# lucidrains/ring-attention-pytorch

Hardware: AMD Instinct MI355X
Metric: attn_tflops (higher is better)
Workload: dtype bf16; 1 GPU; model=ring_flash_attn (non-causal, d_head 64), global_batch=1, seq_len=8192, seq_per_gpu=8192, heads=8, kv_heads=8, d_head=64, parallelism=ring1, hipgraph=True

## Files before the change

ring_attention_amd/csrc/attn_bwd.hip:

```cpp

#include <hip/hip_runtime.h>
#include <hip/hip_bf16.h>
#include <cstdint>

#include "attn_common.h"

namespace ring_attn {

template <int D>
struct DqLds {
    static constexpr int KVB = kvblk(D);
    __align__(16) __bf16 k[2][KVB * D];
    __align__(16) __bf16 v[2][KVB * D];
    unsigned char kmask[2][KVB];
};

template <int D, bool SOFTCLAMP, bool PAIRED, bool BIAS = false>
__global__ __launch_bounds__(512, 2)
void attn_bwd_dq_kernel(BwdParams p) {
    constexpr int DBLK = D / 32;
    constexpr int KSTEPS = D / 16;
    constexpr int DQ_KVBLK = kvblk(D);
    constexpr int DQ_NBLK = DQ_KVBLK / 32;

    __shared__ DqLds<D> lds;

    const int tid = threadIdx.x;
    const int lane = tid & 63;
    const int wid = tid >> 6;
    const int l31 = lane & 31;
    const int lhi = lane >> 5;

    const int bh = blockIdx.y;
    const int b = bh / p.h;
    const int h = bh % p.h;
    const int hk = h % p.hk;

    const int n_pit = PAIRED
        ? (p.paired - 1 - (int)blockIdx.x == (int)blockIdx.x ? 1 : 2) : 1;
    for (int pit = 0; pit < n_pit; ++pit) {
    const int qtile = PAIRED
        ? (pit == 0 ? (int)blockIdx.x : p.paired - 1 - (int)blockIdx.x)
        : (p.desc ? p.desc[(long)blockIdx.x * 3] : (int)blockIdx.x);
    if (PAIRED && pit == 1) {
        __syncthreads();
    }

    auto dq_body = [&]() {
    const BwdParams P = p;
    const long i = (long)qtile * ROWS_WG + wid * 32 + l31;
    const bool row_valid = i < P.nq;
    const long ic = row_valid ? i : 0;

    const __bf16* qbase = (const __bf16*)P.q + ((long)b * P.nq + ic) * P.h * D + (long)h * D;
    const __bf16* dobase = (const __bf16*)P.dout + ((long)b * P.nq + ic) * P.h * D + (long)h * D;
    bf16x8 qf[KSTEPS], dof[KSTEPS];
    #pragma unroll
    for (int ks = 0; ks < KSTEPS; ++ks) {
        qf[ks] = *(const bf16x8*)(qbase + ks * 16 + lhi * 8);
        dof[ks] = *(const bf16x8*)(dobase + ks * 16 + lhi * 8);
    }
    const float lse_i = P.lse[((long)b * P.h + h) * P.nq + ic] * LOG2E;
    const float delta_i = P.delta[((long)b * P.h + h) * P.nq + ic];

    f32x16 dq_acc[DBLK];
    #pragma unroll
    for (int db = 0; db < DBLK; ++db) dq_acc[db] = f32x16{};

    const Mask M = mask_of(P);
    const long wg_i_min = (long)qtile * ROWS_WG;
    const long wg_i_max = min((long)(qtile + 1) * ROWS_WG, P.nq) - 1;
    const long wg_q_min = M.qpos(wg_i_min);
    const long wg_q_max = M.qpos(wg_i_max);
    const long qpos_i = M.qpos(i);
    TileRange tr = M.kv_tile_range(wg_i_min, wg_i_max, P.nk, DQ_KVBLK);
    if (P.split > 1) tr = split_share(tr, P.split, (int)blockIdx.z);
    if (!PAIRED && P.desc)
        tr = {P.desc[(long)blockIdx.x * 3 + 1], P.desc[(long)blockIdx.x * 3 + 2]};
    const int t_lo = tr.lo, t_hi = tr.hi;

    constexpr int CH = D * 2 / 16;
    constexpr int KCHUNKS = DQ_KVBLK * CH;
    constexpr int KREGS = (KCHUNKS + 511) / 512;
    const __bf16* kbase = (const __bf16*)P.k + ((long)b * P.nk) * P.hk * D + (long)hk * D;
    const __bf16* vbase = (const __bf16*)P.v + ((long)b * P.nk) * P.hk * D + (long)hk * D;
    const unsigned char* mbase = P.kmask ? (const unsigned char*)P.kmask + (long)b * P.nk : nullptr;

    const long kv_row_stride = (long)P.hk * D;
    const long tile_stride = DQ_KVBLK * kv_row_stride;
    const __bf16* kptr = kbase + (long)t_lo * tile_stride
        + (tid / CH) * kv_row_stride + (tid % CH) * 8;
    const __bf16* vptr = vbase + (long)t_lo * tile_stride
        + (tid / CH) * kv_row_stride + (tid % CH) * 8;
    long j0_next = (long)t_lo * DQ_KVBLK;

    uint4 kst[KREGS], vst[KREGS];
    unsigned char mst = 1;

    auto load_tile = [&]() {
        const long j0 = j0_next;
        const long jmax = min(j0 + DQ_KVBLK, P.nk) - 1;
        const bool full = jmax - j0 == DQ_KVBLK - 1;
        #pragma unroll
        for (int r = 0; r < KREGS; ++r) {
            int c = tid + r * 512;
            if (c < KCHUNKS) {
                long off = (long)(r * (512 / CH)) * kv_row_stride;
                bool okr = full || (j0 + c / CH) <= jmax;
                kst[r] = okr ? *(const uint4*)(kptr + off) : uint4{0, 0, 0, 0};
                vst[r] = okr ? *(const uint4*)(vptr + off) : uint4{0, 0, 0, 0};
            }
        }
        if (mbase && tid < DQ_KVBLK)
            mst = (j0 + tid <= jmax) ? mbase[j0 + tid] : 0;
        kptr += tile_stride; vptr += tile_stride;
        j0_next += DQ_KVBLK;
    };

    auto write_tile = [&](int par) {
        #pragma unroll
        for (int r = 0; r < KREGS; ++r) {
            int c = tid + r * 512;
            if (c < KCHUNKS) {
                int row = c / CH, ch = c % CH;
                *(uint4*)(lds.k[par] + row * D + swz<D / 8>(row, ch) * 8) = kst[r];
                *(uint4*)(lds.v[par] + row * D + swz<D / 8>(row, ch) * 8) = vst[r];
            }
        }
        if (mbase && tid < DQ_KVBLK) lds.kmask[par][tid] = mst;
    };

    const float scale2 = P.scale * LOG2E;
    if (t_lo < t_hi) {
        load_tile();
        write_tile(t_lo & 1);
        if (t_lo + 1 < t_hi) load_tile();
    }

    for (int t = t_lo; t < t_hi; ++t) {
        const int par = t & 1;
        const long j0 = (long)t * DQ_KVBLK;
        const long jmax = min(j0 + DQ_KVBLK, P.nk) - 1;
        const bool full_tile = !BIAS &&
            (jmax - j0 == DQ_KVBLK - 1) &&
            M.uncut(wg_q_min, wg_q_max, j0, jmax) &&
            !P.kmask;

        __syncthreads();

        alignas(16) uint32_t pk[DQ_NBLK * 8];
        __builtin_amdgcn_s_setprio(1);
        #pragma unroll
        for (int kb = 0; kb < DQ_NBLK; ++kb) {
            f32x16 s = f32x16{}, dp = f32x16{};
            int krow = kb * 32 + l31;
            #pragma unroll
            for (int ks = 0; ks < KSTEPS; ++ks) {
                int chunk = ks * 2 + lhi;
                bf16x8 kfr = *(const bf16x8*)(lds.k[par] + krow * D + swz<D / 8>(krow, chunk) * 8);
                bf16x8 vfr = *(const bf16x8*)(lds.v[par] + krow * D + swz<D / 8>(krow, chunk) * 8);
                s = __builtin_amdgcn_mfma_f32_32x32x16_bf16(kfr, qf[ks], s, 0, 0, 0);
                dp = __builtin_amdgcn_mfma_f32_32x32x16_bf16(vfr, dof[ks], dp, 0, 0, 0);
            }
            if (full_tile && row_valid) {
                #pragma unroll
                for (int x2 = 0; x2 < 8; ++x2) {
                    float dse[2];
                    #pragma unroll
                    for (int e = 0; e < 2; ++e) {
                        int r = 2 * x2 + e;
                        float x, dtanh = 1.f;
                        if constexpr (SOFTCLAMP) {
                            float inv_v = __builtin_amdgcn_rcpf(P.softclamp_value);
                            float th = fast_tanhf(s[r] * P.scale * inv_v);
                            x = P.softclamp_value * th * LOG2E;
                            dtanh = 1.f - th * th;
                        } else {
                            x = __builtin_fmaf(s[r], scale2, -lse_i);
                        }
                        float pv = __builtin_amdgcn_exp2f(SOFTCLAMP ? x - lse_i : x);
                        dse[e] = pv * (dp[r] - delta_i);
                        if constexpr (SOFTCLAMP) dse[e] *= dtanh;
                    }
                    pk[kb * 8 + x2] = pack_bf16x2(dse[0], dse[1]);
                }
            } else {
                #pragma unroll
                for (int x2 = 0; x2 < 8; ++x2) {
                    float dse[2];
                    #pragma unroll
                    for (int e = 0; e < 2; ++e) {
                        int r = 2 * x2 + e;
                        long jj = j0 + kb * 32 + (r & 3) + 8 * (r >> 2) + 4 * lhi;
                        float x, dtanh = 1.f;
                        if constexpr (SOFTCLAMP) {
                            float inv_v = __builtin_amdgcn_rcpf(P.softclamp_value);
                            float th = fast_tanhf(s[r] * P.scale * inv_v);
                            x = P.softclamp_value * th * LOG2E;
                            dtanh = 1.f - th * th;
                        } else {
                            x = s[r] * scale2;
                        }
                        bool ok = row_valid && jj <= jmax;
                        if constexpr (BIAS) {
                            if (ok) {
                                const long bi = P.bias_mat
                                    ? (((long)b * P.h + h) * P.nq + ic) * P.nk + jj
                                    : ((long)b * P.h + h) * P.nk + jj;
                                x += P.bias[bi] * LOG2E;
                            }
                        }
                        ok = M.attends(qpos_i, jj, ok);
                        if (P.kmask) ok = ok && lds.kmask[par][jj - j0];
                        float pv = ok ? __builtin_amdgcn_exp2f(
                            SOFTCLAMP ? x - lse_i : x - lse_i) : 0.f;
                        dse[e] = pv * (dp[r] - delta_i);
                        if constexpr (SOFTCLAMP) dse[e] *= dtanh;
                    }
                    pk[kb * 8 + x2] = pack_bf16x2(dse[0], dse[1]);
                }
            }
        }
        __builtin_amdgcn_s_setprio(0);

        if (t + 1 < t_hi) write_tile(par ^ 1);
        if (t + 2 < t_hi) load_tile();

        {
            const int f15 = lane & 15;
            const int g16 = (lane >> 4) & 1;
            const unsigned kb_lds = (unsigned)(uintptr_t)
                (__attribute__((address_space(3))) __bf16*)lds.k[par];
            __builtin_amdgcn_s_setprio(1);
            unsigned long long ktr[DBLK][DQ_NBLK * 2][2];
            #pragma unroll
            for (int db = 0; db < DBLK; ++db) {
                const int dg = db * 32 + g16 * 16 + 4 * (f15 & 3);
                #pragma unroll
                for (int ks = 0; ks < DQ_NBLK * 2; ++ks) {
                    #pragma unroll
                    for (int half = 0; half < 2; ++half) {
                        const int kv = ks * 16 + 4 * lhi + 8 * half + (f15 >> 2);
                        const int c = (dg / 8) ^ (kv & (CH < 8 ? CH - 1 : 7));
                        const unsigned a = kb_lds
                            + (unsigned)(kv * (D * 2) + c * 16 + (dg % 8) * 2);
                        asm volatile("ds_read_b64_tr_b16 %0, %1"
                                     : "=&v"(ktr[db][ks][half]) : "v"(a) : "memory");
                    }
                }
            }
            asm volatile("s_waitcnt lgkmcnt(0)" ::: "memory");
            __builtin_amdgcn_sched_barrier(0);
            #pragma unroll
            for (int db = 0; db < DBLK; ++db)
                #pragma unroll
                for (int ks = 0; ks < DQ_NBLK * 2; ++ks) {
                    bf16x8 ktf;
                    *(unsigned long long*)&ktf = ktr[db][ks][0];
                    *((unsigned long long*)&ktf + 1) = ktr[db][ks][1];
                    dq_acc[db] = __builtin_amdgcn_mfma_f32_32x32x16_bf16(
                        ktf, *(const bf16x8*)(pk + 4 * ks), dq_acc[db], 0, 0, 0);
                }
            __builtin_amdgcn_s_setprio(0);
        }
    }

    if (!row_valid) return;
    #pragma unroll
    for (int db = 0; db < DBLK; ++db) dq_acc[db] *= P.scale;
    if (P.dq_bf) {
        __bf16* dqb = (__bf16*)P.dq_bf + ((long)b * P.nq + i) * P.h * D + (long)h * D;
        #pragma unroll
        for (int db = 0; db < DBLK; ++db)
            #pragma unroll
            for (int g = 0; g < 4; ++g) {
                f32x4 v4 = {dq_acc[db][4 * g], dq_acc[db][4 * g + 1],
                            dq_acc[db][4 * g + 2], dq_acc[db][4 * g + 3]};
                *(bf16x4*)(dqb + db * 32 + 8 * g + 4 * lhi) =
                    __builtin_convertvector(v4, bf16x4);
            }
        return;
    }
    float* dqp = P.dq + ((long)b * P.nq + i) * P.h * D + (long)h * D;
    #pragma unroll
    for (int db = 0; db < DBLK; ++db)
        #pragma unroll
        for (int r = 0; r < 16; ++r) {
            int d = db * 32 + (r & 3) + 8 * (r >> 2) + 4 * lhi;
            if (P.split > 1 || P.desc) atomicAdd(dqp + d, dq_acc[db][r]);
            else if (P.accumulate) dqp[d] += dq_acc[db][r];
            else dqp[d] = dq_acc[db][r];
        }
    };
    dq_body();
    }
}

static constexpr int KVROWS_WAVE = 32;
static_assert(ROWS_WG == 8 * KVROWS_WAVE);

template <int D, int QT>
struct DkvLds {
    __align__(16) __bf16 q[2][QT * D];
    __align__(16) __bf16 qt[2][D * QT];
    __align__(16) __bf16 do_[2][QT * D];
    __align__(16) __bf16 dot[2][D * QT];
    __align__(16) float lse[2][QT];
    __align__(16) float delta[2][QT];
};


template <int D, int QT, bool SOFTCLAMP, bool PAIRED, bool BIAS = false>
__global__ __launch_bounds__(512, 2)
void attn_bwd_dkv_kernel(BwdParams p) {
    static_assert(D % 32 == 0 && QT % 32 == 0);
    constexpr int DBLK = D / 32;
    constexpr int KSTEPS = D / 16;
    constexpr int QBLKS = QT / 32;
    constexpr int TM = (QT / 8 - 1) < 7 ? (QT / 8 - 1) : 7;

    __shared__ DkvLds<D, QT> lds;

    constexpr bool FRAME = (D == 64);
    constexpr bool PREFETCH = (D == 64);

    const int n_pit = PAIRED
        ? (p.paired - 1 - (int)blockIdx.x == (int)blockIdx.x ? 1 : 2) : 1;
    for (int pit = 0; pit < n_pit; ++pit) {
    const int kvtile_wg = PAIRED
        ? (pit == 0 ? (int)blockIdx.x : p.paired - 1 - (int)blockIdx.x)
        : (p.desc ? p.desc[(long)blockIdx.x * 3] : (int)blockIdx.x);
    if (PAIRED && pit == 1) {
        __syncthreads();
    }

    auto dkv_body = [&](int kvtile_arg, unsigned long long kernarg) {
    const BwdParams P = [&] {
        if constexpr (FRAME) {
            BwdParams kp = kernarg_params<BwdParams>(kernarg);
            kp.q = as_global(kp.q);         kp.k = as_global(kp.k);
            kp.v = as_global(kp.v);         kp.dout = as_global(kp.dout);
            kp.kmask = as_global(kp.kmask); kp.lse = as_global(kp.lse);
            kp.delta = as_global(kp.delta); kp.dk = as_global(kp.dk);
            kp.dv = as_global(kp.dv);       kp.dk_bf = as_global(kp.dk_bf);
            kp.dv_bf = as_global(kp.dv_bf); kp.bias = as_global(kp.bias);
            kp.desc = as_global(kp.desc);
            return kp;
        } else {
            return p;
        }
    }();
    const int kvtile = uniform<FRAME>(kvtile_arg);
    const int tid = threadIdx.x;
    const int lane = tid & 63;
    const int wid = uniform<FRAME>(tid >> 6);
    const int l31 = lane & 31;
    const int lhi = lane >> 5;
    const int bhk = blockIdx.y;
    const int b = bhk / P.hk;
    const int hkh = bhk % P.hk;

    const long j0_wg = (long)kvtile * ROWS_WG;
    const long jmax = min(j0_wg + ROWS_WG, P.nk) - 1;
    const long j = j0_wg + wid * KVROWS_WAVE + l31;
    const bool col_valid = j <= jmax;
    const long jc = col_valid ? j : j0_wg;

    const __bf16* kb = (const __bf16*)P.k + ((long)b * P.nk + jc) * P.hk * D + (long)hkh * D;
    const __bf16* vb = (const __bf16*)P.v + ((long)b * P.nk + jc) * P.hk * D + (long)hkh * D;
    bf16x8 kf[KSTEPS], vf[KSTEPS];
    #pragma unroll
    for (int ks = 0; ks < KSTEPS; ++ks) {
        kf[ks] = *(const bf16x8*)(kb + ks * 16 + lhi * 8);
        vf[ks] = *(const bf16x8*)(vb + ks * 16 + lhi * 8);
    }
    unsigned char kmask_own = 1;
    if (P.kmask) kmask_own = col_valid ? ((const unsigned char*)P.kmask)[(long)b * P.nk + j] : 0;

    f32x16 dv_acc[DBLK], dk_acc[DBLK];
    #pragma unroll
    for (int db = 0; db < DBLK; ++db) { dv_acc[db] = f32x16{}; dk_acc[db] = f32x16{}; }
    const float scale2 = P.scale * LOG2E;

    const Mask M = mask_of(P);

    if constexpr (FRAME) __builtin_amdgcn_s_waitcnt(0x0F70);

    for (int g = 0; g < P.group; ++g) {
        if (g > 0) __syncthreads();
        const int h = hkh + g * P.hk;
        const float* lse_row = P.lse + ((long)b * P.h + h) * P.nq;
        const float* delta_row = P.delta + ((long)b * P.h + h) * P.nq;
        const __bf16* qg = (const __bf16*)P.q + ((long)b * P.nq) * P.h * D + (long)h * D;
        const __bf16* dog = (const __bf16*)P.dout + ((long)b * P.nq) * P.h * D + (long)h * D;

        TileRange tr = M.q_tile_range(j0_wg, jmax, P.nq, QT);
        if (P.split > 1) tr = split_share(tr, P.split, (int)blockIdx.z);
        if (!PAIRED && P.desc)
            tr = {uniform<FRAME>(P.desc[(long)blockIdx.x * 3 + 1]),
                  uniform<FRAME>(P.desc[(long)blockIdx.x * 3 + 2])};
        const int t0 = tr.lo, t1 = tr.hi;

        constexpr int CH = D * 2 / 16;
        constexpr int QCHUNKS = QT * CH;
        constexpr int QREGS = (QCHUNKS + 511) / 512;
        constexpr int TPAIRS = (QT / 2) * (D / 8);
        constexpr int TREGS = (TPAIRS + 511) / 512;
        uint4 qst[QREGS], dost[QREGS];
        bf16x8 qtv_a[TREGS], qtv_b[TREGS], dov_a[TREGS], dov_b[TREGS];
        float lse_st = 0.f, delta_st = 0.f;
        long t_next = t0;

        const unsigned qrow_bytes = (unsigned)(P.h * D) * 2u;
        auto ld16 = [](const __bf16* base, unsigned boff) {
            return *(const uint4*)((const char*)base + boff);
        };
        auto ld8h = [](const __bf16* base, unsigned boff) {
            return *(const bf16x8*)((const char*)base + boff);
        };
        auto tile_rows = [&](long tile) {
            return (int)(min((tile + 1) * QT, P.nq) - tile * QT);
        };
        auto load_qtile = [&](int tid) {
            const long i0 = t_next * QT;
            const int last = tile_rows(t_next) - 1;
            const __bf16* qtile = qg + i0 * P.h * D;
            const __bf16* dotile = dog + i0 * P.h * D;
            #pragma unroll
            for (int r = 0; r < QREGS; ++r) {
                int c = tid + r * 512;
                if (c < QCHUNKS) {
                    int lr = min(c / CH, last);
                    int ch = c % CH;
                    unsigned off = (unsigned)lr * qrow_bytes + ch * 16;
                    qst[r] = ld16(qtile, off);
                    dost[r] = ld16(dotile, off);
                }
            }
            #pragma unroll
            for (int r = 0; r < TREGS; ++r) {
                int c = tid + r * 512;
                if (c < TPAIRS) {
                    int jp = c % (QT / 2);
                    int d0 = (c / (QT / 2)) * 8;
                    unsigned offa = (unsigned)min(jp * 2, last) * qrow_bytes + d0 * 2;
                    unsigned offb = (unsigned)min(jp * 2 + 1, last) * qrow_bytes + d0 * 2;
                    qtv_a[r] = ld8h(qtile, offa);
                    qtv_b[r] = ld8h(qtile, offb);
                    dov_a[r] = ld8h(dotile, offa);
                    dov_b[r] = ld8h(dotile, offb);
                }
            }
            if (tid < QT) {
                long gi = i0 + min(tid, last);
                lse_st = lse_row[gi];
                delta_st = delta_row[gi];
            }
            ++t_next;
        };

        auto write_qtile = [&](int par, int tid, long tile) {
            const int rows = tile_rows(tile);
            if (rows < QT) {
                #pragma unroll
                for (int r = 0; r < QREGS; ++r)
                    if ((tid + r * 512) / CH >= rows) {
                        qst[r] = uint4{0, 0, 0, 0};
                        dost[r] = uint4{0, 0, 0, 0};
                    }
                #pragma unroll
                for (int r = 0; r < TREGS; ++r) {
                    int la = ((tid + r * 512) % (QT / 2)) * 2;
                    if (la >= rows) { qtv_a[r] = bf16x8{}; dov_a[r] = bf16x8{}; }
                    if (la + 1 >= rows) { qtv_b[r] = bf16x8{}; dov_b[r] = bf16x8{}; }
                }
            }
            #pragma unroll
            for (int r = 0; r < QREGS; ++r) {
                int c = tid + r * 512;
                if (c < QCHUNKS) {
                    int row = c / CH, ch = c % CH;
                    *(uint4*)(lds.q[par] + row * D + swz<D / 8>(row, ch) * 8) = qst[r];
                    *(uint4*)(lds.do_[par] + row * D + swz<D / 8>(row, ch) * 8) = dost[r];
                }
            }
            #pragma unroll
            for (int r = 0; r < TREGS; ++r) {
                int c = tid + r * 512;
                if (c < TPAIRS) {
                    int jp = kperm_pair(c % (QT / 2));
                    int d0 = (c / (QT / 2)) * 8;
                    static_assert((TM << 4) < QT * 2 && (D * QT * 2) % (QT * 2) == 0);
                    const unsigned base = par * (D * QT * 2) + d0 * QT * 2 + jp * 4;
                    #pragma unroll
                    for (int e = 0; e < 8; ++e) {
                        unsigned byte_off = (base ^ ((e & TM) << 4)) + e * QT * 2;
                        __bf16 pq[2] = {qtv_a[r][e], qtv_b[r][e]};
                        __bf16 pd[2] = {dov_a[r][e], dov_b[r][e]};
                        *(uint32_t*)((char*)lds.qt[0] + byte_off) = *(uint32_t*)pq;
                        *(uint32_t*)((char*)lds.dot[0] + byte_off) = *(uint32_t*)pd;
                    }
                }
            }
            if (tid < QT) {
                const bool okl = tid < rows;
                lds.lse[par][tid] = okl ? lse_st * LOG2E : 0.f;
                lds.delta[par][tid] = okl ? delta_st : 0.f;
            }
        };

        if (t0 < t1) {
            load_qtile(tid);
            write_qtile(t0 & 1, tid, t0);
            if (t0 + 1 < t1) load_qtile(tid);
        }

        for (int t = t0; t < t1; ++t) {
            const int par = t & 1;
            const long i0 = (long)t * QT;
            const long imax = min(i0 + QT, P.nq) - 1;
            const bool full_tile = !BIAS &&
                (imax - i0 == QT - 1) &&
                M.uncut(M.qpos(i0), M.qpos(imax), j0_wg, jmax) &&
                !P.kmask;

            bf16x8 qa[KSTEPS], da[KSTEPS], doa[2 * DBLK], qta[2 * DBLK];
            auto read_sdp = [&](int qb) {
                #pragma unroll
                for (int ks = 0; ks < KSTEPS; ++ks) {
                    int qrow = qb * 32 + l31;
                    int chunk = ks * 2 + lhi;
                    qa[ks] = *(const bf16x8*)(lds.q[par] + qrow * D + swz<D / 8>(qrow, chunk) * 8);
                    da[ks] = *(const bf16x8*)(lds.do_[par] + qrow * D + swz<D / 8>(qrow, chunk) * 8);
                }
            };
            auto read_dvdk = [&](int qb) {
                #pragma unroll
                for (int db = 0; db < DBLK; ++db)
                    #pragma unroll
                    for (int half = 0; half < 2; ++half) {
                        int qk = qb * 2 + half;
                        int drow = db * 32 + l31;
                        int ch = qk * 2 + lhi;
                        doa[db * 2 + half] = *(const bf16x8*)(lds.dot[par] + drow * QT +
                                                              ((ch ^ (drow & TM))) * 8);
                        qta[db * 2 + half] = *(const bf16x8*)(lds.qt[par] + drow * QT +
                                                              ((ch ^ (drow & TM))) * 8);
                    }
            };

            const int rows_m1 = (int)(imax - i0);
            int lhi4 = 4 * lhi;
            asm volatile("" : "+v"(lhi4));
            long qp_lane = M.qpos(i0 + lhi4);
            asm volatile("" : "+v"(qp_lane));

            __syncthreads();

            if constexpr (PREFETCH) {
                read_sdp(0);
                __builtin_amdgcn_sched_barrier(0);
            }

            int tid_l = tid;
            if constexpr (FRAME) asm volatile("" : "+v"(tid_l));
            if (t + 1 < t1) write_qtile(par ^ 1, tid_l, t + 1);
            if (t + 2 < t1) load_qtile(tid_l);

            #pragma unroll
            for (int qb = 0; qb < QBLKS; ++qb) {
                f32x16 s2 = f32x16{}, dp = f32x16{};
                if constexpr (!PREFETCH) read_sdp(qb);
                #pragma unroll
                for (int ks = 0; ks < KSTEPS; ++ks) {
                    s2 = __builtin_amdgcn_mfma_f32_32x32x16_bf16(qa[ks], kf[ks], s2, 0, 0, 0);
                    dp = __builtin_amdgcn_mfma_f32_32x32x16_bf16(da[ks], vf[ks], dp, 0, 0, 0);
                }
                f32x4 lse_g0 = f32x4{}, delta_g0 = f32x4{};
                if constexpr (PREFETCH) {
                    lse_g0 = *(const f32x4*)(lds.lse[par] + qb * 32 + 4 * lhi);
                    delta_g0 = *(const f32x4*)(lds.delta[par] + qb * 32 + 4 * lhi);
                    read_dvdk(qb);
                    __builtin_amdgcn_sched_barrier(0);
                }

                alignas(16) uint32_t p_pk[8], ds_pk[8];
                if (full_tile && col_valid) {
                    #pragma unroll
                    for (int x2 = 0; x2 < 8; ++x2) {
                        float pe[2], dse[2];
                        f32x4 lse4, delta4;
                        if (PREFETCH && (x2 >> 1) == 0) {
                            lse4 = lse_g0;
                            delta4 = delta_g0;
                        } else {
                            int base = qb * 32 + 8 * (x2 >> 1) + 4 * lhi;
                            lse4 = *(const f32x4*)(lds.lse[par] + base);
                            delta4 = *(const f32x4*)(lds.delta[par] + base);
                        }
                        #pragma unroll
                        for (int e = 0; e < 2; ++e) {
                            int r = 2 * x2 + e;
                            float x, dtanh = 1.f;
                            if constexpr (SOFTCLAMP) {
                                float inv_v = __builtin_amdgcn_rcpf(P.softclamp_value);
                                float th = fast_tanhf(s2[r] * P.scale * inv_v);
                                x = P.softclamp_value * th * LOG2E;
                                dtanh = 1.f - th * th;
                            } else {
                                x = __builtin_fmaf(s2[r], scale2, -lse4[r & 3]);
                            }
                            float pv = __builtin_amdgcn_exp2f(SOFTCLAMP ? x - lse4[r & 3] : x);
                            pe[e] = pv;
                            dse[e] = pv * (dp[r] - delta4[r & 3]);
                            if constexpr (SOFTCLAMP) dse[e] *= dtanh;
                        }
                        p_pk[x2] = pack_bf16x2(pe[0], pe[1]);
                        ds_pk[x2] = pack_bf16x2(dse[0], dse[1]);
                    }
                } else {
                    #pragma unroll
                    for (int x2 = 0; x2 < 8; ++x2) {
                        float pe[2], dse[2];
                        f32x4 lse4, delta4;
                        if (PREFETCH && (x2 >> 1) == 0) {
                            lse4 = lse_g0;
                            delta4 = delta_g0;
                        } else {
                            int base = qb * 32 + 8 * (x2 >> 1) + 4 * lhi;
                            lse4 = *(const f32x4*)(lds.lse[par] + base);
                            delta4 = *(const f32x4*)(lds.delta[par] + base);
                        }
                        #pragma unroll
                        for (int e = 0; e < 2; ++e) {
                            int r = 2 * x2 + e;
                            const int cr = qb * 32 + (r & 3) + 8 * (r >> 2);
                            const int qloc = cr + lhi4;
                            float x, dtanh = 1.f;
                            if constexpr (SOFTCLAMP) {
                                float inv_v = __builtin_amdgcn_rcpf(P.softclamp_value);
                                float th = fast_tanhf(s2[r] * P.scale * inv_v);
                                x = P.softclamp_value * th * LOG2E;
                                dtanh = 1.f - th * th;
                            } else {
                                x = s2[r] * scale2;
                            }
                            bool ok = col_valid && qloc <= rows_m1;
                            if constexpr (BIAS) {
                                if (ok) {
                                    const long i = i0 + qloc;
                                    const long bi = P.bias_mat
                                        ? (((long)b * P.h + h) * P.nq + i) * P.nk + j
                                        : ((long)b * P.h + h) * P.nk + j;
                                    x += P.bias[bi] * LOG2E;
                                }
                            }
                            ok = M.attends(qp_lane + (long)cr * M.q_stride, j, ok);
                            if (P.kmask) ok = ok && kmask_own;
                            float pv = ok ? __builtin_amdgcn_exp2f(x - lse4[r & 3]) : 0.f;
                            pe[e] = pv;
                            dse[e] = pv * (dp[r] - delta4[r & 3]);
                            if constexpr (SOFTCLAMP) dse[e] *= dtanh;
                        }
                        p_pk[x2] = pack_bf16x2(pe[0], pe[1]);
                        ds_pk[x2] = pack_bf16x2(dse[0], dse[1]);
                    }
                }

                if constexpr (PREFETCH) {
                    if (qb + 1 < QBLKS) {
                        read_sdp(qb + 1);
                        __builtin_amdgcn_sched_barrier(0);
                    }
                } else {
                    read_dvdk(qb);
                }
                #pragma unroll
                for (int db = 0; db < DBLK; ++db)
                    #pragma unroll
                    for (int half = 0; half < 2; ++half) {
                        dv_acc[db] = __builtin_amdgcn_mfma_f32_32x32x16_bf16(
                            doa[db * 2 + half], *(const bf16x8*)(p_pk + 4 * half), dv_acc[db], 0, 0, 0);
                        dk_acc[db] = __builtin_amdgcn_mfma_f32_32x32x16_bf16(
                            *(const bf16x8*)(ds_pk + 4 * half), qta[db * 2 + half], dk_acc[db], 0, 0, 0);
                    }
            }
        }
    }

    #pragma unroll
    for (int db = 0; db < DBLK; ++db) dk_acc[db] *= P.scale;

    if (P.dk_bf) {
        constexpr int ECH = D / 8;
        __bf16* stg_dk = (__bf16*)&lds;
        __bf16* stg_dv = stg_dk + ROWS_WG * D;
        static_assert(sizeof(DkvLds<D, QT>) >= 2 * ROWS_WG * D * sizeof(__bf16));
        const int wrow0 = wid * KVROWS_WAVE;
        const long orow_stride = (long)P.hk * D;
        __bf16* dkb = (__bf16*)P.dk_bf + ((long)b * P.nk) * orow_stride + (long)hkh * D;
        __bf16* dvb = (__bf16*)P.dv_bf + ((long)b * P.nk) * orow_stride + (long)hkh * D;
        __syncthreads();
        #pragma unroll
        for (int db = 0; db < DBLK; ++db)
            #pragma unroll
            for (int r = 0; r < 16; ++r) {
                int row = wrow0 + (r & 3) + 8 * (r >> 2) + 4 * lhi;
                int d = db * 32 + l31;
                stg_dk[row * D + swz<ECH>(row, d / 8) * 8 + (d & 7)] = (__bf16)dk_acc[db][r];
            }
        {
            const int row = wrow0 + l31;
            #pragma unroll
            for (int db = 0; db < DBLK; ++db)
                #pragma unroll
                for (int g = 0; g < 4; ++g) {
                    f32x4 v4 = {dv_acc[db][4 * g], dv_acc[db][4 * g + 1],
                                dv_acc[db][4 * g + 2], dv_acc[db][4 * g + 3]};
                    *(bf16x4*)(stg_dv + row * D + swz<ECH>(row, db * 4 + g) * 8 + 4 * lhi) =
                        __builtin_convertvector(v4, bf16x4);
                }
        }
        __syncthreads();
        #pragma unroll
        for (int c = lane; c < KVROWS_WAVE * ECH; c += 64) {
            int row = wrow0 + c / ECH, ch = c % ECH;
            long kvrow = j0_wg + row;
            if (kvrow <= jmax) {
                int so = row * D + swz<ECH>(row, ch) * 8;
                *(uint4*)(dkb + kvrow * orow_stride + ch * 8) = *(const uint4*)(stg_dk + so);
                *(uint4*)(dvb + kvrow * orow_stride + ch * 8) = *(const uint4*)(stg_dv + so);
            }
        }
    } else {
        float* dkb = P.dk + (((long)b * P.hk + hkh) * P.nk) * D;
        #pragma unroll
        for (int db = 0; db < DBLK; ++db)
            #pragma unroll
            for (int r = 0; r < 16; ++r) {
                long kvrow = j0_wg + wid * KVROWS_WAVE + (r & 3) + 8 * (r >> 2) + 4 * lhi;
                int d = db * 32 + l31;
                if (kvrow <= jmax) {
                    float* dst = dkb + kvrow * D + d;
                    if (P.split > 1 || P.desc) atomicAdd(dst, dk_acc[db][r]);
                    else if (P.accumulate) *dst += dk_acc[db][r];
                    else *dst = dk_acc[db][r];
                }
            }
        float* dvb = P.dv + (((long)b * P.hk + hkh) * D) * P.nk;
        if (col_valid)
        #pragma unroll
        for (int db = 0; db < DBLK; ++db)
            #pragma unroll
            for (int r = 0; r < 16; ++r) {
                int d = db * 32 + (r & 3) + 8 * (r >> 2) + 4 * lhi;
                float* dst = dvb + (long)d * P.nk + j;
                if (P.split > 1 || P.desc) atomicAdd(dst, dv_acc[db][r]);
                else if (P.accumulate) *dst += dv_acc[db][r];
                else *dst = dv_acc[db][r];
            }
    }
    };
    if constexpr (FRAME) noinline_call(dkv_body, kvtile_wg, kernarg_address());
    else dkv_body(kvtile_wg, 0ull);
    }
}

void launch_attn_bwd_dq(const BwdParams& p, int head_dim, hipStream_t stream) {
    dim3 block(512);
    int z = p.split > 1 ? p.split : 1;
    long qt_ = ceil_div(p.nq, ROWS_WG);
    if (p.desc) qt_ = p.n_units;
    else if (p.paired) qt_ = (qt_ + 1) / 2;
    dim3 grid_dq(qt_, p.b * p.h, z);
    const bool pr = p.paired > 0;
    if (p.bias) {
        if (head_dim == 64) {
            if (p.softclamp) hipLaunchKernelGGL((attn_bwd_dq_kernel<64, true, false, true>), grid_dq, block, 0, stream, p);
            else hipLaunchKernelGGL((attn_bwd_dq_kernel<64, false, false, true>), grid_dq, block, 0, stream, p);
        } else if (head_dim == 128) {
            if (p.softclamp) hipLaunchKernelGGL((attn_bwd_dq_kernel<128, true, false, true>), grid_dq, block, 0, stream, p);
            else hipLaunchKernelGGL((attn_bwd_dq_kernel<128, false, false, true>), grid_dq, block, 0, stream, p);
        } else {
            if (p.softclamp) hipLaunchKernelGGL((attn_bwd_dq_kernel<32, true, false, true>), grid_dq, block, 0, stream, p);
            else hipLaunchKernelGGL((attn_bwd_dq_kernel<32, false, false, true>), grid_dq, block, 0, stream, p);
        }
        return;
    }
    if (head_dim == 64) {
        if (p.softclamp) if (pr) hipLaunchKernelGGL((attn_bwd_dq_kernel<64, true, true>), grid_dq, block, 0, stream, p);
        else hipLaunchKernelGGL((attn_bwd_dq_kernel<64, true, false>), grid_dq, block, 0, stream, p);
        else if (pr) hipLaunchKernelGGL((attn_bwd_dq_kernel<64, false, true>), grid_dq, block, 0, stream, p);
        else hipLaunchKernelGGL((attn_bwd_dq_kernel<64, false, false>), grid_dq, block, 0, stream, p);
    } else if (head_dim == 128) {
        if (p.softclamp) if (pr) hipLaunchKernelGGL((attn_bwd_dq_kernel<128, true, true>), grid_dq, block, 0, stream, p);
        else hipLaunchKernelGGL((attn_bwd_dq_kernel<128, true, false>), grid_dq, block, 0, stream, p);
        else if (pr) hipLaunchKernelGGL((attn_bwd_dq_kernel<128, false, true>), grid_dq, block, 0, stream, p);
        else hipLaunchKernelGGL((attn_bwd_dq_kernel<128, false, false>), grid_dq, block, 0, stream, p);
    } else if (head_dim == 32) {
        if (p.softclamp) if (pr) hipLaunchKernelGGL((attn_bwd_dq_kernel<32, true, true>), grid_dq, block, 0, stream, p);
        else hipLaunchKernelGGL((attn_bwd_dq_kernel<32, true, false>), grid_dq, block, 0, stream, p);
        else if (pr) hipLaunchKernelGGL((attn_bwd_dq_kernel<32, false, true>), grid_dq, block, 0, stream, p);
        else hipLaunchKernelGGL((attn_bwd_dq_kernel<32, false, false>), grid_dq, block, 0, stream, p);
    } else {
        __builtin_trap();
    }
}

void launch_attn_bwd_dkv(const BwdParams& p, int head_dim, hipStream_t stream) {
    dim3 block(512);
    int z = p.split > 1 ? p.split : 1;
    long kt_ = ceil_div(p.nk, ROWS_WG);
    if (p.desc) kt_ = p.n_units;
    else if (p.paired) kt_ = (kt_ + 1) / 2;
    dim3 grid_dkv(kt_, p.b * p.hk, z);
    const bool pr = p.paired > 0;
    if (p.bias) {
        if (head_dim == 64) {
            if (p.softclamp) hipLaunchKernelGGL((attn_bwd_dkv_kernel<64, DKV_QT, true, false, true>), grid_dkv, block, 0, stream, p);
            else hipLaunchKernelGGL((attn_bwd_dkv_kernel<64, DKV_QT, false, false, true>), grid_dkv, block, 0, stream, p);
        } else if (head_dim == 128) {
            if (p.softclamp) hipLaunchKernelGGL((attn_bwd_dkv_kernel<128, DKV_QT, true, false, true>), grid_dkv, block, 0, stream, p);
            else hipLaunchKernelGGL((attn_bwd_dkv_kernel<128, DKV_QT, false, false, true>), grid_dkv, block, 0, stream, p);
        } else {
            if (p.softclamp) hipLaunchKernelGGL((attn_bwd_dkv_kernel<32, DKV_QT, true, false, true>), grid_dkv, block, 0, stream, p);
            else hipLaunchKernelGGL((attn_bwd_dkv_kernel<32, DKV_QT, false, false, true>), grid_dkv, block, 0, stream, p);
        }
        return;
    }
    if (head_dim == 64) {
        if (p.softclamp) if (pr) hipLaunchKernelGGL((attn_bwd_dkv_kernel<64, DKV_QT, true, true>), grid_dkv, block, 0, stream, p);
        else hipLaunchKernelGGL((attn_bwd_dkv_kernel<64, DKV_QT, true, false>), grid_dkv, block, 0, stream, p);
        else if (pr) hipLaunchKernelGGL((attn_bwd_dkv_kernel<64, DKV_QT, false, true>), grid_dkv, block, 0, stream, p);
        else hipLaunchKernelGGL((attn_bwd_dkv_kernel<64, DKV_QT, false, false>), grid_dkv, block, 0, stream, p);
    } else if (head_dim == 128) {
        if (p.softclamp) if (pr) hipLaunchKernelGGL((attn_bwd_dkv_kernel<128, DKV_QT, true, true>), grid_dkv, block, 0, stream, p);
        else hipLaunchKernelGGL((attn_bwd_dkv_kernel<128, DKV_QT, true, false>), grid_dkv, block, 0, stream, p);
        else if (pr) hipLaunchKernelGGL((attn_bwd_dkv_kernel<128, DKV_QT, false, true>), grid_dkv, block, 0, stream, p);
        else hipLaunchKernelGGL((attn_bwd_dkv_kernel<128, DKV_QT, false, false>), grid_dkv, block, 0, stream, p);
    } else if (head_dim == 32) {
        if (p.softclamp) if (pr) hipLaunchKernelGGL((attn_bwd_dkv_kernel<32, DKV_QT, true, true>), grid_dkv, block, 0, stream, p);
        else hipLaunchKernelGGL((attn_bwd_dkv_kernel<32, DKV_QT, true, false>), grid_dkv, block, 0, stream, p);
        else if (pr) hipLaunchKernelGGL((attn_bwd_dkv_kernel<32, DKV_QT, false, true>), grid_dkv, block, 0, stream, p);
        else hipLaunchKernelGGL((attn_bwd_dkv_kernel<32, DKV_QT, false, false>), grid_dkv, block, 0, stream, p);
    } else {
        __builtin_trap();
    }
}

template <int D>
__global__ __launch_bounds__(256) void attn_delta_kernel(DeltaParams p) {
    constexpr int LPR = D / 8;
    constexpr int RPW = 64 / LPR;
    const int lane = threadIdx.x & 63;
    const int wave = (blockIdx.x * (blockDim.x >> 6)) + (threadIdx.x >> 6);
    const long row = (long)wave * RPW + lane / LPR;
    if (row >= p.rows) return;
    const int c = lane % LPR;

    const __bf16* dop = (const __bf16*)p.dout + row * D + c * 8;
    const __bf16* op = (const __bf16*)p.out + row * D + c * 8;
    bf16x8 a = *(const bf16x8*)dop;
    bf16x8 b = *(const bf16x8*)op;
    float s = 0.f;
    #pragma unroll
    for (int e = 0; e < 8; ++e) s += (float)a[e] * (float)b[e];
    #pragma unroll
    for (int off = LPR / 2; off > 0; off >>= 1) s += __shfl_xor(s, off);
    if (c == 0) {
        const long hh = row % p.h;
        const long bi = row / p.h;
        const long i = bi % p.n, bb = bi / p.n;
        p.delta[(bb * p.h + hh) * p.n + i] = s;
    }
}

void launch_attn_delta(const DeltaParams& p, int head_dim, hipStream_t stream) {
    dim3 block(256);
    if (head_dim == 64) {
        long waves = (p.rows + 7) / 8;
        hipLaunchKernelGGL(attn_delta_kernel<64>, dim3((waves + 3) / 4), block, 0, stream, p);
    } else if (head_dim == 128) {
        long waves = (p.rows + 3) / 4;
        hipLaunchKernelGGL(attn_delta_kernel<128>, dim3((waves + 3) / 4), block, 0, stream, p);
    } else if (head_dim == 32) {
        long waves = (p.rows + 15) / 16;
        hipLaunchKernelGGL(attn_delta_kernel<32>, dim3((waves + 3) / 4), block, 0, stream, p);
    } else {
        __builtin_trap();
    }
}

static constexpr int FIN_ROWS = 64;

__device__ __forceinline__ uint4 fin_pack8(const float* s) {
    f32x4 a = {s[0], s[1], s[2], s[3]}, c = {s[4], s[5], s[6], s[7]};
    union { bf16x4 h[2]; uint4 u; } o;
    o.h[0] = __builtin_convertvector(a, bf16x4);
    o.h[1] = __builtin_convertvector(c, bf16x4);
    return o.u;
}

template <int D>
__global__ __launch_bounds__(256) void attn_bwd_finalize_kernel(BwdFinalizeParams p) {
    constexpr int CH = D / 8;
    constexpr int LDW = FIN_ROWS + 1;
    __shared__ float tile[D * LDW];
    const int tid = threadIdx.x;
    const int which = blockIdx.z;

    if (which == 2) {
        if (!p.dq) return;
        const long nblk = (long)gridDim.x * gridDim.y;
        const long blk = (long)blockIdx.y * gridDim.x + blockIdx.x;
        const long chunks = p.dq_elems / 8;
        for (long c = blk * 256 + tid; c < chunks; c += nblk * 256) {
            float s[8];
            *(f32x4*)s = *(const f32x4*)(p.dq + c * 8);
            *(f32x4*)(s + 4) = *(const f32x4*)(p.dq + c * 8 + 4);
            *(uint4*)((__bf16*)p.dq_bf + c * 8) = fin_pack8(s);
        }
        return;
    }
    if (!p.dk) return;

    const int bb = blockIdx.y / p.hk;
    const int hh = blockIdx.y % p.hk;
    const long n0 = (long)blockIdx.x * FIN_ROWS;
    const int rows = (int)min((long)FIN_ROWS, p.nk - n0);
    const long orow_stride = (long)p.hk * D;

    if (which == 0) {
        const float* src = p.dk + (((long)bb * p.hk + hh) * p.nk + n0) * D;
        __bf16* dst = (__bf16*)p.dk_bf + ((long)bb * p.nk + n0) * orow_stride + (long)hh * D;
        for (int c = tid; c < rows * CH; c += 256) {
            int row = c / CH, ch = c % CH;
            float s[8];
            *(f32x4*)s = *(const f32x4*)(src + (long)row * D + ch * 8);
            *(f32x4*)(s + 4) = *(const f32x4*)(src + (long)row * D + ch * 8 + 4);
            *(uint4*)(dst + row * orow_stride + ch * 8) = fin_pack8(s);
        }
        return;
    }

    const float* src = p.dv + (((long)bb * p.hk + hh) * D) * p.nk + n0;
    for (int c = tid; c < D * FIN_ROWS; c += 256) {
        int d = c / FIN_ROWS, nn = c % FIN_ROWS;
        if (nn < rows) tile[d * LDW + nn] = src[(long)d * p.nk + nn];
    }
    __syncthreads();
    __bf16* dst = (__bf16*)p.dv_bf + ((long)bb * p.nk + n0) * orow_stride + (long)hh * D;
    for (int c = tid; c < rows * CH; c += 256) {
        int row = c / CH, ch = c % CH;
        float s[8];
        #pragma unroll
        for (int e = 0; e < 8; ++e) s[e] = tile[(ch * 8 + e) * LDW + row];
        *(uint4*)(dst + row * orow_stride + ch * 8) = fin_pack8(s);
    }
}

void launch_attn_bwd_finalize(const BwdFinalizeParams& p, int head_dim, hipStream_t stream) {
    dim3 block(256);
    long nx = p.dk ? (p.nk + FIN_ROWS - 1) / FIN_ROWS : 256;
    int ny = p.dk ? p.b * p.hk : 1;
    dim3 grid(nx, ny, p.dq ? 3 : 2);
    if (head_dim == 64) hipLaunchKernelGGL(attn_bwd_finalize_kernel<64>, grid, block, 0, stream, p);
    else if (head_dim == 128) hipLaunchKernelGGL(attn_bwd_finalize_kernel<128>, grid, block, 0, stream, p);
    else if (head_dim == 32) hipLaunchKernelGGL(attn_bwd_finalize_kernel<32>, grid, block, 0, stream, p);
    else __builtin_trap();
}

}
```

ring_attention_amd/csrc/attn_common.h:

```cpp
#pragma once

#include <hip/hip_runtime.h>
#include <cstdint>

#ifdef __HIPCC__
#include <hip/hip_bf16.h>
#endif

#include "attn_mask.h"

namespace ring_attn {

#ifdef __HIPCC__
typedef __bf16 bf16_t;
typedef bf16_t bf16x8 __attribute__((ext_vector_type(8)));
typedef float f32x16 __attribute__((ext_vector_type(16)));
typedef float f32x4 __attribute__((ext_vector_type(4)));
typedef bf16_t bf16x4 __attribute__((ext_vector_type(4)));
typedef unsigned int u32x2 __attribute__((ext_vector_type(2)));
typedef float f32x2 __attribute__((ext_vector_type(2)));
typedef bf16_t bf16x2 __attribute__((ext_vector_type(2)));

__device__ __forceinline__ uint32_t pack_bf16x2(float a, float b) {
    union { bf16x2 h; uint32_t u; } c;
    c.h = __builtin_convertvector(f32x2{a, b}, bf16x2);
    return c.u;
}

__device__ __forceinline__ int kperm_pair(int jp) {
    return (jp & ~6) | ((jp & 4) >> 1) | ((jp & 2) << 1);
}

template <int CH>
__device__ __forceinline__ int swz(int row, int chunk) {
    return chunk ^ (row & (CH < 8 ? CH - 1 : 7));
}

__device__ __forceinline__ float fast_tanhf(float x) {
    float e = __builtin_amdgcn_exp2f(x * 2.885390081777927f);
    return 1.f - 2.f * __builtin_amdgcn_rcpf(e + 1.f);
}

__device__ __forceinline__ float cross_half(float x) {
    union { float f; unsigned u; } c; c.f = x;
    u32x2 r = __builtin_amdgcn_permlane32_swap(c.u, c.u, false, false);
    union { unsigned u; float f; } lo, hi; lo.u = r[0]; hi.u = r[1];
    return (threadIdx.x & 32) ? lo.f : hi.f;
}

template <class F>
__device__ __attribute__((noinline)) void noinline_call(F&& f) { f(); }

template <class F>
__device__ __attribute__((noinline, not_tail_called))
void noinline_call(F&& f, int x, unsigned long long kernarg) { f(x, kernarg); }

template <bool ON>
__device__ __forceinline__ int uniform(int x) {
    if constexpr (ON) return __builtin_amdgcn_readfirstlane(x);
    else return x;
}

__device__ __forceinline__ unsigned long long kernarg_address() {
    return (unsigned long long)__builtin_amdgcn_kernarg_segment_ptr();
}

template <class T>
__device__ __forceinline__ T kernarg_params(unsigned long long kernarg) {
    static_assert(sizeof(T) % 4 == 0);
    typedef const __attribute__((address_space(4))) unsigned int* const_words;
    const unsigned lo = __builtin_amdgcn_readfirstlane((unsigned)kernarg);
    const unsigned hi = __builtin_amdgcn_readfirstlane((unsigned)(kernarg >> 32));
    const_words src = (const_words)(((unsigned long long)hi << 32) | lo);
    union { T t; unsigned w[sizeof(T) / 4]; } u;
    #pragma unroll
    for (unsigned i = 0; i < sizeof(T) / 4; ++i) u.w[i] = src[i];
    return u.t;
}

template <class T>
__device__ __forceinline__ T* as_global(T* p) {
    return (T*)(__attribute__((address_space(1))) T*)(unsigned long long)p;
}

static constexpr float LOG2E = 1.4426950408889634f;
static constexpr float LN2 = 0.6931471805599453f;
#endif

static constexpr float MASK_VALUE_F = -3.4028234663852886e38f;

struct FwdParams {
    const void* q;
    const void* k;
    const void* v;
    const void* kmask;
    float* o_acc;
    float* m;
    float* l;
    void* out;
    float* lse;
    int b, h, hk, group;
    long nq, nk;
    float scale;
    float softclamp_value;
    int softclamp;
    int causal;
    long diag;
    long q_stride;
    long win;
    int has_win;
    int is_first;
    int is_last;
    int kv_split;
    int ablate;
    int paired;
    unsigned long long* ticks;
    const float* bias;
    int bias_mat;
};

struct FwdMergeParams {
    const float* o_part;
    const float* m_part;
    const float* l_part;
    float* o_acc;
    float* m;
    float* l;
    void* out;
    float* lse;
    int splits;
    int b, h;
    long nq;
    int is_first;
    int is_last;
};

void launch_attn_fwd_merge(const FwdMergeParams& p, int head_dim, hipStream_t stream);

void launch_attn_fwd(const FwdParams& p, int head_dim, hipStream_t stream);

bool launch_attn_fwd_v2(const FwdParams& p, int head_dim, hipStream_t stream);

struct BwdParams {
    const void* q;
    const void* k;
    const void* v;
    const void* dout;
    const void* kmask;
    const float* lse;
    const float* delta;
    float* dq;
    float* dk;
    float* dv;
    void* dq_bf;
    void* dk_bf;
    void* dv_bf;
    int b, h, hk, group;
    long nq, nk;
    float scale;
    float softclamp_value;
    int softclamp;
    int causal;
    long diag;
    long q_stride;
    long win;
    int has_win;
    int accumulate;
    int split;
    int paired;
    const float* bias;
    int bias_mat;
    const int* desc;
    long n_units;
};

void launch_attn_bwd_dq(const BwdParams& p, int head_dim, hipStream_t stream);
void launch_attn_bwd_dkv(const BwdParams& p, int head_dim, hipStream_t stream);

struct BwdFinalizeParams {
    const float* dk;
    const float* dv;
    const float* dq;
    void* dk_bf;
    void* dv_bf;
    void* dq_bf;
    int b, hk;
    long nk;
    long dq_elems;
};

void launch_attn_bwd_finalize(const BwdFinalizeParams& p, int head_dim, hipStream_t stream);

struct DeltaParams {
    const void* dout;
    const void* out;
    float* delta;
    long rows;
    long n;
    int h;
};

void launch_attn_delta(const DeltaParams& p, int head_dim, hipStream_t stream);

struct DecodeParams {
    const void* q;
    const void* k;
    const void* v;
    float* out;
    float* lse;
    int b, h;
    int hk;
    int nq;
    long n;
    float scale;
    long chunks;
    const void* kscale;
    const void* vscale;
};

void launch_decode_partial(const DecodeParams& p, int head_dim, hipStream_t stream);
void launch_decode_partial_fp8(const DecodeParams& p, int head_dim, hipStream_t stream);

struct DecodeMergeParams {
    const float* outs;
    const float* lses;
    float* out;
    float* lse;
    long rows;
    int s;
};

void launch_decode_merge(const DecodeMergeParams& p, int head_dim, hipStream_t stream);

struct PagedDecodeParams {
    const void* q;
    const void* k_pages;
    const void* v_pages;
    const void* kscale;
    const void* vscale;
    const int* block_table;
    const int* seq_lens;
    float* out;
    float* lse;
    int b, h;
    int hk;
    int nq;
    int page_shift;
    int max_pages;
    int num_pages;
    int causal;
    int chunk_major;
    float scale;
    long chunks;
    long max_seq_len;
};

void launch_decode_partial_paged(const PagedDecodeParams& p, int head_dim, bool fp8,
                                 hipStream_t stream);

struct PagedAppendParams {
    const void* k_new;
    const void* v_new;
    void* k_pages;
    void* v_pages;
    void* kscale;
    void* vscale;
    const int* block_table;
    const int* seq_lens;
    const int* append_lens;
    int b, hk, t;
    int page_shift, max_pages, num_pages;
};

void launch_paged_kv_append(const PagedAppendParams& p, int head_dim, bool fp8,
                            hipStream_t stream);

struct PagedPrefillParams {
    const void* q;
    const void* k_pages;
    const void* v_pages;
    const void* kscale;
    const void* vscale;
    const int* block_table;
    const int* seq_lens;
    const int* q_lens;
    float* o_part;
    float* m_part;
    float* l_part;
    void* out;
    float* lse;
    int b, h, hk;
    int t;
    int page_shift, max_pages, num_pages;
    int causal, has_win;
    long win;
    float scale;
    int kv_split;
};

void launch_attn_fwd_paged(const PagedPrefillParams& p, int head_dim, bool fp8,
                           hipStream_t stream);

struct Fp8FwdCore {
    const void* q;
    const void* k;
    const void* vt;
    const void* qs;
    const void* ks;
    const void* vs;
    void* out;
    float* lse;
    int b, h, hk;
    long nq, nk;
    long nk_true;
    int nvs;
    float scale;
    int causal;
    int paired;
};

struct Fp8FwdParams : Fp8FwdCore {
    int has_win;
    long diag, q_stride, win;
};

void launch_attn_fwd_fp8(const Fp8FwdParams& p, int head_dim, hipStream_t stream);

struct RotaryParams {
    const void* x;
    const float* cos_t;
    const float* sin_t;
    void* out;
    long rows;
    int n, h, d;
    float sin_sign;
};

void launch_rotary(const RotaryParams& p, int head_dim, hipStream_t stream);

}
```

Before: 446.4 TFLOP/s.

## Use ds_read_tr transposed LDS reads in dK/dV bwd instead of separate transposed images

For head dims other than 128, the dK/dV backward kernel no longer builds transposed copies of Q and dO in LDS. It reads the normal row-major tiles with ds_read_tr16_b64 transposing loads. This removes the register staging, global reloads and scattered LDS stores needed for the transposed images, and halves the LDS footprint, with padding kept so the bf16 epilogue staging still fits. Separately, some float sub/mul ops are wrapped in empty asm barriers to stop the compiler from contracting or reordering them, which may change the instruction schedule.

Result: faster. 472.1 TFLOP/s (median of 6 runs) (+5.8%).

```diff
diff --git a/ring_attention_amd/csrc/attn_bwd.hip b/ring_attention_amd/csrc/attn_bwd.hip
--- a/ring_attention_amd/csrc/attn_bwd.hip
+++ b/ring_attention_amd/csrc/attn_bwd.hip
@@ -179,8 +179,8 @@
                             x = __builtin_fmaf(s[r], scale2, -lse_i);
                         }
                         float pv = __builtin_amdgcn_exp2f(SOFTCLAMP ? x - lse_i : x);
-                        dse[e] = pv * (dp[r] - delta_i);
-                        if constexpr (SOFTCLAMP) dse[e] *= dtanh;
+                        dse[e] = mul_f32(pv, sub_f32(dp[r], delta_i));
+                        if constexpr (SOFTCLAMP) dse[e] = mul_f32(dse[e], dtanh);
                     }
                     pk[kb * 8 + x2] = pack_bf16x2(dse[0], dse[1]);
                 }
@@ -214,8 +214,8 @@
                         if (P.kmask) ok = ok && lds.kmask[par][jj - j0];
                         float pv = ok ? __builtin_amdgcn_exp2f(
                             SOFTCLAMP ? x - lse_i : x - lse_i) : 0.f;
-                        dse[e] = pv * (dp[r] - delta_i);
-                        if constexpr (SOFTCLAMP) dse[e] *= dtanh;
+                        dse[e] = mul_f32(pv, sub_f32(dp[r], delta_i));
+                        if constexpr (SOFTCLAMP) dse[e] = mul_f32(dse[e], dtanh);
                     }
                     pk[kb * 8 + x2] = pack_bf16x2(dse[0], dse[1]);
                 }
@@ -267,7 +267,9 @@
 
     if (!row_valid) return;
     #pragma unroll
-    for (int db = 0; db < DBLK; ++db) dq_acc[db] *= P.scale;
+    for (int db = 0; db < DBLK; ++db)
+        #pragma unroll
+        for (int r = 0; r < 16; ++r) dq_acc[db][r] = mul_f32(dq_acc[db][r], P.scale);
     if (P.dq_bf) {
         __bf16* dqb = (__bf16*)P.dq_bf + ((long)b * P.nq + i) * P.h * D + (long)h * D;
         #pragma unroll
@@ -299,7 +301,7 @@
 static constexpr int KVROWS_WAVE = 32;
 static_assert(ROWS_WG == 8 * KVROWS_WAVE);
 
-template <int D, int QT>
+template <int D, int QT, bool SINGLE_IMAGE>
 struct DkvLds {
     __align__(16) __bf16 q[2][QT * D];
     __align__(16) __bf16 qt[2][D * QT];
@@ -309,6 +311,23 @@
     __align__(16) float delta[2][QT];
 };
 
+template <int D, int QT>
+struct DkvLds<D, QT, true> {
+    __align__(16) __bf16 q[2][QT * D];
+    __align__(16) __bf16 do_[2][QT * D];
+    __align__(16) float lse[2][QT];
+    __align__(16) float delta[2][QT];
+    __align__(16) __bf16 epilogue_room[2 * ROWS_WG * D - 4 * QT * D];
+    static_assert(2 * ROWS_WG * D > 4 * QT * D);
+};
+
+
+template <int TREGS, bool TWO_IMAGE>
+struct DkvTrStage {
+    bf16x8 q_a[TREGS], q_b[TREGS], do_a[TREGS], do_b[TREGS];
+};
+template <int TREGS>
+struct DkvTrStage<TREGS, false> {};
 
 template <int D, int QT, bool SOFTCLAMP, bool PAIRED, bool BIAS = false>
 __global__ __launch_bounds__(512, 2)
@@ -319,7 +338,8 @@
     constexpr int QBLKS = QT / 32;
     constexpr int TM = (QT / 8 - 1) < 7 ? (QT / 8 - 1) : 7;
 
-    __shared__ DkvLds<D, QT> lds;
+    constexpr bool SINGLE_IMAGE = (D != 128);
+    __shared__ DkvLds<D, QT, SINGLE_IMAGE> lds;
 
     constexpr bool FRAME = (D == 64);
     constexpr bool PREFETCH = (D == 64);
@@ -407,7 +427,7 @@
         constexpr int TPAIRS = (QT / 2) * (D / 8);
         constexpr int TREGS = (TPAIRS + 511) / 512;
         uint4 qst[QREGS], dost[QREGS];
-        bf16x8 qtv_a[TREGS], qtv_b[TREGS], dov_a[TREGS], dov_b[TREGS];
+        DkvTrStage<TREGS, !SINGLE_IMAGE> trs;
         float lse_st = 0.f, delta_st = 0.f;
         long t_next = t0;
 
@@ -437,18 +457,20 @@
                     dost[r] = ld16(dotile, off);
                 }
             }
-            #pragma unroll
-            for (int r = 0; r < TREGS; ++r) {
-                int c = tid + r * 512;
-                if (c < TPAIRS) {
-                    int jp = c % (QT / 2);
-                    int d0 = (c / (QT / 2)) * 8;
-                    unsigned offa = (unsigned)min(jp * 2, last) * qrow_bytes + d0 * 2;
-                    unsigned offb = (unsigned)min(jp * 2 + 1, last) * qrow_bytes + d0 * 2;
-                    qtv_a[r] = ld8h(qtile, offa);
-                    qtv_b[r] = ld8h(qtile, offb);
-                    dov_a[r] = ld8h(dotile, offa);
-                    dov_b[r] = ld8h(dotile, offb);
+            if constexpr (!SINGLE_IMAGE) {
+                #pragma unroll
+                for (int r = 0; r < TREGS; ++r) {
+                    int c = tid + r * 512;
+                    if (c < TPAIRS) {
+                        int jp = c % (QT / 2);
+                        int d0 = (c / (QT / 2)) * 8;
+                        unsigned offa = (unsigned)min(jp * 2, last) * qrow_bytes + d0 * 2;
+                        unsigned offb = (unsigned)min(jp * 2 + 1, last) * qrow_bytes + d0 * 2;
+                        trs.q_a[r] = ld8h(qtile, offa);
+                        trs.q_b[r] = ld8h(qtile, offb);
+                        trs.do_a[r] = ld8h(dotile, offa);
+                        trs.do_b[r] = ld8h(dotile, offb);
+                    }
                 }
             }
             if (tid < QT) {
@@ -468,11 +490,13 @@
                         qst[r] = uint4{0, 0, 0, 0};
                         dost[r] = uint4{0, 0, 0, 0};
                     }
-                #pragma unroll
-                for (int r = 0; r < TREGS; ++r) {
-                    int la = ((tid + r * 512) % (QT / 2)) * 2;
-                    if (la >= rows) { qtv_a[r] = bf16x8{}; dov_a[r] = bf16x8{}; }
-                    if (la + 1 >= rows) { qtv_b[r] = bf16x8{}; dov_b[r] = bf16x8{}; }
+                if constexpr (!SINGLE_IMAGE) {
+                    #pragma unroll
+                    for (int r = 0; r < TREGS; ++r) {
+                        int la = ((tid + r * 512) % (QT / 2)) * 2;
+                        if (la >= rows) { trs.q_a[r] = bf16x8{}; trs.do_a[r] = bf16x8{}; }
+                        if (la + 1 >= rows) { trs.q_b[r] = bf16x8{}; trs.do_b[r] = bf16x8{}; }
+                    }
                 }
             }
             #pragma unroll
@@ -484,21 +508,23 @@
                     *(uint4*)(lds.do_[par] + row * D + swz<D / 8>(row, ch) * 8) = dost[r];
                 }
             }
-            #pragma unroll
-            for (int r = 0; r < TREGS; ++r) {
-                int c = tid + r * 512;
-                if (c < TPAIRS) {
-                    int jp = kperm_pair(c % (QT / 2));
-                    int d0 = (c / (QT / 2)) * 8;
-                    static_assert((TM << 4) < QT * 2 && (D * QT * 2) % (QT * 2) == 0);
-                    const unsigned base = par * (D * QT * 2) + d0 * QT * 2 + jp * 4;
-                    #pragma unroll
-                    for (int e = 0; e < 8; ++e) {
-                        unsigned byte_off = (base ^ ((e & TM) << 4)) + e * QT * 2;
-                        __bf16 pq[2] = {qtv_a[r][e], qtv_b[r][e]};
-                        __bf16 pd[2] = {dov_a[r][e], dov_b[r][e]};
-                        *(uint32_t*)((char*)lds.qt[0] + byte_off) = *(uint32_t*)pq;
-                        *(uint32_t*)((char*)lds.dot[0] + byte_off) = *(uint32_t*)pd;
+            if constexpr (!SINGLE_IMAGE) {
+                #pragma unroll
+                for (int r = 0; r < TREGS; ++r) {
+                    int c = tid + r * 512;
+                    if (c < TPAIRS) {
+                        int jp = kperm_pair(c % (QT / 2));
+                        int d0 = (c / (QT / 2)) * 8;
+                        static_assert((TM << 4) < QT * 2 && (D * QT * 2) % (QT * 2) == 0);
+                        const unsigned base = par * (D * QT * 2) + d0 * QT * 2 + jp * 4;
+                        #pragma unroll
+                        for (int e = 0; e < 8; ++e) {
+                            unsigned byte_off = (base ^ ((e & TM) << 4)) + e * QT * 2;
+                            __bf16 pq[2] = {trs.q_a[r][e], trs.q_b[r][e]};
+                            __bf16 pd[2] = {trs.do_a[r][e], trs.do_b[r][e]};
+                            *(uint32_t*)((char*)lds.qt[0] + byte_off) = *(uint32_t*)pq;
+                            *(uint32_t*)((char*)lds.dot[0] + byte_off) = *(uint32_t*)pd;
+                        }
                     }
                 }
             }
@@ -534,19 +560,51 @@
                     da[ks] = *(const bf16x8*)(lds.do_[par] + qrow * D + swz<D / 8>(qrow, chunk) * 8);
                 }
             };
-            auto read_dvdk = [&](int qb) {
-                #pragma unroll
-                for (int db = 0; db < DBLK; ++db)
+            auto read_dvdk_tr = [&](int qb) {
+                typedef __attribute__((address_space(3))) bf16x4* lds_v4;
+                const int f15 = lane & 15;
+                const int g16 = (lane >> 4) & 1;
+                const int lrow = 4 * lhi + (f15 >> 2);
+                const int key = lrow & (D / 8 < 8 ? D / 8 - 1 : 7);
+                #pragma unroll
+                for (int db = 0; db < DBLK; ++db) {
+                    const int col = db * 32 + 16 * g16 + 4 * (f15 & 3);
+                    const int lane_off = lrow * D + ((col / 8) ^ key) * 8 + (col % 8);
                     #pragma unroll
                     for (int half = 0; half < 2; ++half) {
-                        int qk = qb * 2 + half;
-                        int drow = db * 32 + l31;
-                        int ch = qk * 2 + lhi;
-                        doa[db * 2 + half] = *(const bf16x8*)(lds.dot[par] + drow * QT +
-                                                              ((ch ^ (drow & TM))) * 8);
-                        qta[db * 2 + half] = *(const bf16x8*)(lds.qt[par] + drow * QT +
-                                                              ((ch ^ (drow & TM))) * 8);
-                    }
+                        bf16x4 dv4[2], qv4[2];
+                        #pragma unroll
+                        for (int u = 0; u < 2; ++u) {
+                            const int off = (qb * 32 + 16 * half + 8 * u) * D + lane_off;
+                            dv4[u] = __builtin_amdgcn_ds_read_tr16_b64_v4bf16(
+                                (lds_v4)(lds.do_[par] + off));
+                            qv4[u] = __builtin_amdgcn_ds_read_tr16_b64_v4bf16(
+                                (lds_v4)(lds.q[par] + off));
+                        }
+                        doa[db * 2 + half] = __builtin_shufflevector(
+                            dv4[0], dv4[1], 0, 1, 2, 3, 4, 5, 6, 7);
+                        qta[db * 2 + half] = __builtin_shufflevector(
+                            qv4[0], qv4[1], 0, 1, 2, 3, 4, 5, 6, 7);
+                    }
+                }
+            };
+            auto read_dvdk = [&](int qb) {
+                if constexpr (SINGLE_IMAGE) {
+                    read_dvdk_tr(qb);
+                } else {
+                    #pragma unroll
+                    for (int db = 0; db < DBLK; ++db)
+                        #pragma unroll
+                        for (int half = 0; half < 2; ++half) {
+                            int qk = qb * 2 + half;
+                            int drow = db * 32 + l31;
+                            int ch = qk * 2 + lhi;
+                            doa[db * 2 + half] = *(const bf16x8*)(lds.dot[par] + drow * QT +
+                                                                  ((ch ^ (drow & TM))) * 8);
+                            qta[db * 2 + half] = *(const bf16x8*)(lds.qt[par] + drow * QT +
+                                                                  ((ch ^ (drow & TM))) * 8);
+                        }
+                }
             };
 
             const int rows_m1 = (int)(imax - i0);
@@ -612,8 +670,8 @@
                             }
                             float pv = __builtin_amdgcn_exp2f(SOFTCLAMP ? x - lse4[r & 3] : x);
                             pe[e] = pv;
-                            dse[e] = pv * (dp[r] - delta4[r & 3]);
-                            if constexpr (SOFTCLAMP) dse[e] *= dtanh;
+                            dse[e] = mul_f32(pv, sub_f32(dp[r], delta4[r & 3]));
+                            if constexpr (SOFTCLAMP) dse[e] = mul_f32(dse[e], dtanh);
                         }
                         p_pk[x2] = pack_bf16x2(pe[0], pe[1]);
                         ds_pk[x2] = pack_bf16x2(dse[0], dse[1]);
@@ -659,8 +717,8 @@
                             if (P.kmask) ok = ok && kmask_own;
                             float pv = ok ? __builtin_amdgcn_exp2f(x - lse4[r & 3]) : 0.f;
                             pe[e] = pv;
-                            dse[e] = pv * (dp[r] - delta4[r & 3]);
-                            if constexpr (SOFTCLAMP) dse[e] *= dtanh;
+                            dse[e] = mul_f32(pv, sub_f32(dp[r], delta4[r & 3]));
+                            if constexpr (SOFTCLAMP) dse[e] = mul_f32(dse[e], dtanh);
                         }
                         p_pk[x2] = pack_bf16x2(pe[0], pe[1]);
                         ds_pk[x2] = pack_bf16x2(dse[0], dse[1]);
@@ -689,13 +747,15 @@
     }
 
     #pragma unroll
-    for (int db = 0; db < DBLK; ++db) dk_acc[db] *= P.scale;
+    for (int db = 0; db < DBLK; ++db)
+        #pragma unroll
+        for (int r = 0; r < 16; ++r) dk_acc[db][r] = mul_f32(dk_acc[db][r], P.scale);
 
     if (P.dk_bf) {
         constexpr int ECH = D / 8;
         __bf16* stg_dk = (__bf16*)&lds;
         __bf16* stg_dv = stg_dk + ROWS_WG * D;
-        static_assert(sizeof(DkvLds<D, QT>) >= 2 * ROWS_WG * D * sizeof(__bf16));
+        static_assert(sizeof(DkvLds<D, QT, SINGLE_IMAGE>) >= 2 * ROWS_WG * D * sizeof(__bf16));
         const int wrow0 = wid * KVROWS_WAVE;
         const long orow_stride = (long)P.hk * D;
         __bf16* dkb = (__bf16*)P.dk_bf + ((long)b * P.nk) * orow_stride + (long)hkh * D;
diff --git a/ring_attention_amd/csrc/attn_common.h b/ring_attention_amd/csrc/attn_common.h
--- a/ring_attention_amd/csrc/attn_common.h
+++ b/ring_attention_amd/csrc/attn_common.h
@@ -34,6 +34,17 @@
 template <int CH>
 __device__ __forceinline__ int swz(int row, int chunk) {
     return chunk ^ (row & (CH < 8 ? CH - 1 : 7));
+}
+
+__device__ __forceinline__ float sub_f32(float a, float b) {
+    float r = a - b;
+    asm("" : "+v"(r));
+    return r;
+}
+__device__ __forceinline__ float mul_f32(float a, float b) {
+    float r = a * b;
+    asm("" : "+v"(r));
+    return r;
 }
 
 __device__ __forceinline__ float fast_tanhf(float x) {
```
